# trifectatechfoundation/zlib-rs

Measured on NVIDIA H100. Metric: deflate_level6_raw_input_throughput_silesia_small_tar, higher is better.
Workload: dtype u8

## Files before the change

### __graft_entry__.py

```python
import os
import subprocess
import sys

ROOT = os.path.dirname(os.path.abspath(__file__))
if ROOT not in sys.path:
    sys.path.insert(0, ROOT)
sys.path.insert(0, os.path.join(ROOT, "tests"))


def build():
    subprocess.check_call(["make", "-C", os.path.join(ROOT, "zlib_rs_b200", "csrc"), "-j8"])
    subprocess.check_call(["make", "-C", os.path.join(ROOT, "oracle")])
    subprocess.check_call(["make", "-C", os.path.join(ROOT, "oracle"), "ref"])
    subprocess.check_call(["make", "-C", os.path.join(ROOT, "tests", "hostmodel")])
    subprocess.check_call(["make", "-C", os.path.join(ROOT, "tests", "shardmodel")])
    subprocess.check_call(["make", "-C", os.path.join(ROOT, "tests", "membermodel")])
    subprocess.check_call(["make", "-C", os.path.join(ROOT, "tests", "bgzfmodel")])
    subprocess.check_call(["make", "-C", os.path.join(ROOT, "tests", "c_client")])
    import zlib_rs_b200
    zlib_rs_b200.lib()


def smoke():
    import zlib
    import zlib_rs_b200 as Z
    import oracle_lib as O
    from corpus import synthetic_mix
    d = synthetic_mix(300000, seed=1)
    out = Z.compress2(d, 6)
    assert out == O.compress(d, 6)[1], "GPU deflate differs from the oracle"
    assert zlib.decompress(out) == d
    assert Z.uncompress(out, len(d)) == d
    assert Z.crc32(d) == O.crc32(d) and Z.adler32(d) == O.adler32(d)
    print("smoke ok: %d -> %d bytes, bit-exact vs oracle" % (len(d), len(out)))


if __name__ == "__main__":
    build()
    if len(sys.argv) > 1 and sys.argv[1] == "smoke":
        smoke()
```

### zlib_rs_b200/csrc/zb_core.h

```cpp
#pragma once
#include <stdint.h>

#if defined(__CUDACC__)
#define ZB_HD __host__ __device__ __forceinline__
#define ZB_HDN __host__ __device__
#else
#define ZB_HD inline
#define ZB_HDN
#endif

namespace zb {

constexpr uint32_t kWSize = 32768;
constexpr uint32_t kMaxDist = kWSize - 262;
constexpr uint32_t kMinLookahead = 262;
constexpr uint32_t kT0 = 2 * kWSize - 262;
constexpr uint32_t kMaxMatch = 258;
constexpr uint32_t kLitBufsize = 16384;
constexpr uint32_t kBlockSyms = kLitBufsize - 1;
constexpr uint32_t kTailZone = 1024;
constexpr uint32_t kMSafe = 640;
constexpr uint32_t kPad = 1024;

struct LevelParams {
    uint32_t good, lazy, nice, chain;
    uint32_t early_exit;
};
ZB_HD LevelParams level_params(int level)
{
    switch (level) {
    case 3: return {4, 6, 16, 6, 1};
    case 4: return {4, 12, 32, 24, 1};
    case 5: return {8, 16, 32, 32, 0};
    default: return {8, 16, 128, 128, 0};
    }
}

ZB_HD uint32_t hash_u32(uint32_t v) { return (v * 2654435761u) >> 16; }

struct FullWin {
    ZB_HD uint32_t wsize() const { return kWSize; }
    ZB_HD uint32_t maxdist() const { return kMaxDist; }
    ZB_HD uint32_t t0() const { return kT0; }
};
struct DynWin {
    uint32_t w;
    ZB_HD uint32_t wsize() const { return w; }
    ZB_HD uint32_t maxdist() const { return w - kMinLookahead; }
    ZB_HD uint32_t t0() const { return 2 * w - kMinLookahead; }
};
template <class WN>
ZB_HD uint32_t wbase_w(const WN &wn, uint32_t p) { return p <= wn.t0() ? 0u : wn.wsize() * (1u + (p - wn.t0() - 1u) / wn.wsize()); }

ZB_HD uint32_t wbase(uint32_t p) { return p <= kT0 ? 0u : kWSize * (1u + (p - kT0 - 1u) / kWSize); }

// ... 271 lines not shown
```

### zlib_rs_b200/csrc/zb_engine.cu

```cuda
#include <cuda_runtime.h>
#include <stdio.h>
#include <stdlib.h>
#include <string.h>
#include <new>
#include "../../include/zb_engine.h"
#include "zb_kernels.cuh"
#include "zb_engine_internal.h"

namespace zb {

constexpr uint32_t kSlowSub9 = 24576;
constexpr uint32_t kTailTiles = 2;
constexpr uint32_t kTailSub = 512;

thread_local char g_err[256] = "";

static void set_err(const char *what, cudaError_t e)
{
    snprintf(g_err, sizeof g_err, "%s: %s", what, cudaGetErrorString(e));
}

#define CK(call)                                                  \
    do {                                                          \
        cudaError_t e_ = (call);                                  \
        if (e_ != cudaSuccess) { set_err(#call, e_); return ZB_E_CUDA; } \
    } while (0)

__global__ void k_match(JobBufs);
__global__ void k_skip(JobBufs);
__global__ void k_nxt(JobBufs);
__global__ void k_path_tiles(JobBufs);
__global__ void k_path_chain(JobBufs, uint32_t, uint32_t);
__global__ void k_path_groups(JobBufs, uint32_t, uint32_t, uint4 *, uint32_t *);
__global__ void k_path_chain2(JobBufs, uint32_t, uint32_t, const uint4 *, uint32_t *, uint32_t *);
__global__ void k_path_mark(JobBufs, const uint32_t *, const uint32_t *);
__global__ void k_iter_lists(JobBufs, uint32_t *, uint32_t *, uint32_t);
__global__ void k_emit(JobBufs);
__global__ void k_holes(JobBufs, uint32_t);
__global__ void k_holes_cmp(JobBufs, uint32_t, uint32_t);
__global__ void k_tail(JobBufs);
__global__ void k_block_hist(JobBufs, uint32_t *);
__global__ void k_build_blocks(JobBufs, const uint32_t *);
__global__ void k_scan_blocks(JobBufs);
__global__ void k_encode(JobBufs);
__global__ void k_finish(JobBufs, const uint32_t *);
__global__ void k_literal_syms(JobBufs);
__global__ void k_stored(JobBufs);
__global__ void k_links2_std(JobBufs, uint32_t);
__global__ void k_links2_roll(JobBufs, uint32_t);
__global__ void k_links_fix_std(JobBufs);
__global__ void k_links_fix_roll(JobBufs);
__global__ void k_slow(JobBufs);
__global__ void k_rle(JobBufs);
__global__ void k_emit_slow(JobBufs);
__global__ void k_tail_slow(JobBufs);
__global__ void k_serial_low(JobBufs);
__global__ void k_links_dict_ghost(JobBufs, uint32_t *);
__global__ void k_links_dict_ghost_apply(JobBufs, const uint32_t *);
__global__ void k_bgzf_setup(BgzfJob, uint64_t);
__global__ void k_serial_low_members(JobBufs, BgzfJob);
__global__ void k_bgzf_medium(JobBufs, BgzfJob);
__global__ void k_bgzf_slow_steps(JobBufs, BgzfJob);
__global__ void k_bgzf_slow_walk(JobBufs, BgzfJob);
__global__ void k_bgzf_hist(JobBufs, BgzfJob, uint32_t *);
__global__ void k_bgzf_build(JobBufs, BgzfJob, const uint32_t *);
__global__ void k_bgzf_size(JobBufs, BgzfJob);
__global__ void k_bgzf_scan(JobBufs, BgzfJob);
__global__ void k_bgzf_encode(JobBufs, BgzfJob);
// ... 193 lines not shown
    RES(S_PCNT, ((size_t)N + 16) * 4, pcnt, uint32_t *)
    RES(S_SYMIDX, ((size_t)N + 16) * 4, symidx, uint32_t *)
    RES(S_PHEAD, (size_t)npt * kPathHead * 8, phead, uint2 *)
    RES(S_TENTRY, (size_t)npt * 4, tile_entry, uint32_t *)
    RES(S_TSYMB, (size_t)npt * 4, tile_symbase, uint32_t *)
    RES(S_MARKN, (size_t)npt + 16, mark_needed, uint8_t *)
    const uint32_t nlists = npt * (kPathTile / kPathSub);
    RES(S_LLIST, (size_t)nlists * kLongPerSub * 4, long_list, uint32_t *)
    RES(S_LCNT, (size_t)nlists * 4, long_cnt, uint32_t *)
    RES(S_TDIRTY, (size_t)nmt + 16, tile_dirty, uint8_t *)
    RES(S_SYMS, ((size_t)N + 64) * sizeof(Sym), syms, Sym *)
    RES(S_SYMB, 40000 * 4, sym_base, uint32_t *)
    RES(S_BMAP, (size_t)nmt * 8192, bucket_map, uint32_t *)
    RES(S_LR, npad * 2, Lr, uint16_t *)
    RES(S_KEYS, npad * 2, keys, uint16_t *)
    RES(S_LLAST, (size_t)nmt * 65536 * 2, link_last, uint16_t *)
    RES(S_CSTATE, (size_t)(npt + 1) * 16, chain_state, uint4 *)
    uint32_t chainG = 16;
    while ((uint64_t)chainG * chainG < npt) chainG += 8;
    const uint32_t chain_groups = (npt + chainG - 1) / chainG;
    const uint32_t chain2_smem = chainG * kPathHead * 8 + chain_groups * kPathHead * 16 + chainG * 8;
    const bool chain2 = chain2_smem <= kChain2MaxSmem;
    if ((rc = reserve(S_GFN, (size_t)chain_groups * kPathHead * 16 + ((size_t)npt + 4) * 4, &p)) != ZB_OK) return rc;
    uint4 *d_gfn = static_cast<uint4 *>(p);
    uint32_t *d_mark_cnt = reinterpret_cast<uint32_t *>(d_gfn + (size_t)chain_groups * kPathHead);
    uint32_t *d_mark_list = d_mark_cnt + 4;
    auto launch_chain = [&](uint32_t first_tile) {
        if (chain2) {
            k_path_groups<<<chain_groups, 1024, chainG * kPathHead * 8, st>>>(jb, npt, chainG, d_gfn, d_mark_cnt);
            k_path_chain2<<<chain_groups, 1024, chain2_smem, st>>>(jb, npt, chainG, d_gfn, d_mark_list, d_mark_cnt);
            launches++;
        } else k_path_chain<<<1, 1024, kChainSmemBytes, st>>>(jb, npt, first_tile);
    };
    auto launch_mark = [&](uint32_t grid) {
        if (chain2) k_path_mark<<<grid < npt ? grid : npt, 1024, kPathSmemBytes, st>>>(jb, d_mark_list, d_mark_cnt);
        else k_path_mark<<<npt, 1024, kPathSmemBytes, st>>>(jb, nullptr, nullptr);
    };
    uint32_t *d_lists;
    const uint32_t max_list = N / 512 + 2;
    if ((rc = reserve(S_LISTS, ((size_t)max_list + npt + nmt + 8) * 4, &p)) != ZB_OK) return rc;
    d_lists = static_cast<uint32_t *>(p);
    RES(S_HDIFF, (size_t)nwords * 8, hdiff, uint32_t *)
    jb.hdiff_words = nwords;
    RES(S_HCOARSE, (size_t)(N >> 10) + 16, hcoarse, uint8_t *)
    RES(S_MCHG, (((size_t)N >> 8) + 16) * 4 + 64, mchg, uint8_t *)
    RES(S_BLOCKS, (size_t)max_blocks * sizeof(BlockDesc), blocks, BlockDesc *)
    RES(S_BBASE, (size_t)max_blocks * 4, block_base, uint32_t *)
    uint32_t *d_freq;
    if ((rc = reserve(S_FREQ, (size_t)max_blocks * 320 * 4, &p)) != ZB_OK) return rc;
    d_freq = static_cast<uint32_t *>(p);
    uint8_t *d_out;
    if (dst_dev && dst_cap >= out_cap) d_out = static_cast<uint8_t *>(dst);
    else { if ((rc = reserve(S_OUT, out_cap + 16, &p)) != ZB_OK) return rc; d_out = static_cast<uint8_t *>(p); }
    jb.out = d_out;
    jb.out_cap = out_cap;
    void *d_ck;
    const size_t ck_bytes = ((size_t)N / 16384 + 16) * 8;
    if ((rc = reserve(S_CK, ck_bytes, &d_ck)) != ZB_OK) return rc;
#undef RES
    jb.info = d_info;
    jb.level = (uint32_t)level;
    jb.strategy_fixed = strategy == 4;
    const bool lf_zero = strategy >= 2;
    jb.wrap = wrap;
    jb.hdr_len = wrap == 1 ? 2 : wrap == 2 ? 10 : 0;
    jb.huffman_only = strategy == 2 && level != 0;
// ... 89 lines not shown
                cudaStreamWaitEvent(st, evc[k], 0);
                if (k + 1 < up_chunks) t_hi = up_len[k] >= 64 ? (uint32_t)((up_len[k] - 64) / kLinkTile) : 0;
            }
            if (t_hi <= t_done) continue;
            if (roll) k_links2_roll<<<t_hi - t_done, 1024, kLinks2SmemBytes, st>>>(jb, t_done);
            else k_links2_std<<<t_hi - t_done, 1024, kLinks2SmemBytes, st>>>(jb, t_done);
            if (k) launches++;
            t_done = t_hi;
        }
        if (chunked_upload) cudaStreamWaitEvent(st, evk, 0);
    };
    uint32_t iters = 0;
    if (level == 0) {
        const uint32_t nb = n_in == 0 ? 1 : (uint32_t)((n_in + 65534) / 65535);
        k_stored<<<nb, 256, 0, st>>>(jb);
        launches++;
        k_finish<<<1, 32, 0, st>>>(jb, d_check);
        launches++;
    } else {
        if (jb.huffman_only) {
            k_literal_syms<<<(uint32_t)(n_in / 256 + 1), 256, 0, st>>>(jb);
            launches++;
        } else if (jb.serial_mode) {
            iters = 1;
            pbegin();
            k_serial_low<<<1, 32, jb.serial_mode == 2 ? kSerialSmemBytes : kSerialSmemQuick, st>>>(jb);
            launches++;
            pend(1, 1);
        } else {
            CK(cudaMemsetAsync(jb.holes, 0, (size_t)nwords * 4, st));
            CK(cudaMemsetAsync(jb.holes_new, 0, (size_t)nwords * 4, st));
            CK(cudaMemsetAsync(jb.tile_dirty, 1, nmt, st));
            CK(cudaMemsetAsync(jb.tile_entry, 0xee, (size_t)npt * 4, st));
            CK(cudaMemsetAsync(jb.M + N, 0, (size_t)kPad * 4, st));
            CK(cudaMemsetAsync(jb.L + N, 0, (size_t)kPad * 2, st));
            pbegin();
            if (jb.slow_mode == 2) {
            } else if (jb.slow_mode && jb.sp.slow) {
                links_tiles(true);
                k_links_fix_roll<<<N / 256 + 1, 256, 0, st>>>(jb);
                launches += 2;
            } else {
                links_tiles(false);
                k_links_fix_std<<<N / 256 + 1, 256, 0, st>>>(jb);
                launches += 2;
                if (dstart >= 3 && n_in) {
                    uint32_t *d_first = reinterpret_cast<uint32_t *>(d_check) + 2;
                    CK(cudaMemsetAsync(d_first, 0xff, 4, st));
                    k_links_dict_ghost<<<(kMaxDist + 255) / 256, 256, 0, st>>>(jb, d_first);
                    k_links_dict_ghost_apply<<<1, 32, 0, st>>>(jb, d_first);
                    launches += 2;
                }
            }
            if (!jb.slow_mode) CK(cudaMemcpyAsync(jb.Lr, jb.L, npad * 2, cudaMemcpyDeviceToDevice, st));
            pend(0, 1);
            if (jb.slow_mode) {
                if (n_in > 0) {
                    iters = 1;
                    pbegin();
                    if (jb.slow_mode == 2) k_rle<<<(N + 255) / 256, 256, 0, st>>>(jb);
                    else {
                        jb.match_sub = level >= 9 ? kSlowSub9 : level == 8 ? 4096u : 8192u;
                        k_slow<<<(N + jb.match_sub - 1) / jb.match_sub, 1024, (kWSize + jb.match_sub + kSlowAhead) * 3, st>>>(jb);
                    }
                    pend(1, 1);
                    if (profile) phase_ms[11] = phase_ms[1];
                    pbegin();
                    k_path_tiles<<<npt, 1024, kPathSmemBytes, st>>>(jb);
                    launch_chain(0);
                    launch_mark(npt);
                    pend(3, 3);
                    pbegin();
                    k_emit_slow<<<(N + 255) / 256, 256, 0, st>>>(jb);
                    pend(4, 1);
                    launches += 5;
                }
                pbegin();
                k_tail_slow<<<1, 32, 0, st>>>(jb);
                launches++;
                pend(5, 1);
            } else {
            if (jb.tail_start > 0) {
                uint32_t n_dirty = nmt;
                for (;;) {
                    iters++;
                    uint32_t mthreads = 1024;
                    if (iters == 1) jb.match_sub = 4096;
                    else if (n_dirty <= kTailTiles) { jb.match_sub = kTailSub; mthreads = 256; }
                    else {
                        const uint64_t per_cta = (uint64_t)n_dirty * kMatchTile / (4 * (uint64_t)device_sm_count());
                        jb.match_sub = per_cta >= 8192 ? 8192 : per_cta >= 4096 ? 4096 : per_cta >= 2048 ? 2048 : 1024;
                    }
                    uint32_t nsub = (N + jb.match_sub - 1) / jb.match_sub;
                    uint32_t n_ptiles = npt, first_ptile = 0;
                    jb.skip_list = nullptr;
                    jb.nxt_list = nullptr;
                    if (iters > 1) {
                        jb.skip_list = d_lists;
                        jb.nxt_list = d_lists + nmt + 8;
                        n_ptiles = h_info->n_ptiles ? h_info->n_ptiles : 1;
                        first_ptile = h_info->first_ptile;
                        nsub = (n_dirty ? n_dirty : 1) * (kMatchTile / jb.match_sub);
                        if (n_dirty) {
                            pbegin();
                            k_skip<<<n_dirty, 1024, kSkipSmemBytes, st>>>(jb);
                            pend(1, 1);
                            launches++;
                        }
                    }
                    const uint32_t msmem = (kWSize + jb.match_sub + 512) + (kWSize + jb.match_sub) * 2 +
                                           (iters > 1 ? ((kWSize + jb.match_sub) / 32 + 1) * 4 * 4 + 8192 : 64);
                    jb.use_bucket_map = iters > 1;
                    pbegin();
                    k_match<<<nsub, mthreads, msmem, st>>>(jb);
                    pend(1, 1);
                    if (profile && iters == 1) phase_ms[11] = phase_ms[1];
                    pbegin();
                    k_nxt<<<n_ptiles * (kPathTile / 1024), 1024, 0, st>>>(jb);
                    pend(2, 1);
                    pbegin();
                    k_path_tiles<<<n_ptiles, 1024, kPathSmemBytes, st>>>(jb);
                    launch_chain(first_ptile);
                    launch_mark(iters == 1 ? npt : 2 * n_ptiles + 16);
                    pend(3, 3);
                    pbegin();
                    k_holes<<<(nlists * kLongPerSub + 255) / 256, 256, 0, st>>>(jb, nlists);
                    k_holes_cmp<<<(nwords + 255) / 256, 256, 0, st>>>(jb, nwords, nmt);
                    pend(4, 2);
                    launches += 7;
                    k_iter_lists<<<1, 1024, 0, st>>>(jb, d_lists, d_lists + nmt + 8, npt);
                    launches++;
                    CK(cudaMemcpyAsync(h_info, d_info, sizeof(JobInfo), cudaMemcpyDeviceToHost, st));
                    CK(cudaStreamSynchronize(st));
                    if (h_info->error) { snprintf(g_err, sizeof g_err, "engine error flags 0x%x (parse)", h_info->error); return ZB_E_INTERNAL; }
                    if (getenv("ZB_DEBUG")) {
                        static unsigned long long last[3];
                        if (iters == 1) memset(last, 0, sizeof last);
                        const double ctas = (double)(h_info->dbg[0] - last[0]) + 1e-9;
                        fprintf(stderr, "iter %u dirty %u: ctas %llu stage %.1f walk %.1f kcyc/cta, holes_changed %u, sub %u first_tile %u chain %u\n",
                                iters, n_dirty, h_info->dbg[0] - last[0], (h_info->dbg[1] - last[1]) / 1e3 / ctas,
                                (h_info->dbg[2] - last[2]) / 1e3 / ctas, h_info->holes_changed, jb.match_sub, first_ptile, chain2 ? 2u : 1u);
                        memcpy(last, h_info->dbg, sizeof last);
                    }
                    if (!h_info->holes_changed) break;
                    n_dirty = h_info->n_dirty;
                    if (iters > N / 257u + 4096u) { snprintf(g_err, sizeof g_err, "hole iteration did not converge"); return ZB_E_INTERNAL; }
                }
            }
            CK(cudaEventRecord(evf, st));
            CK(cudaStreamWaitEvent(st2, evf, 0));
            k_tail<<<1, 32, 0, st2>>>(jb);
            launches++;
            CK(cudaEventRecord(evt, st2));
            if (jb.tail_start > 0) {
                pbegin();
                k_emit<<<(jb.tail_start + 255) / 256, 256, 0, st>>>(jb);
                launches++;
                pend(4, 1);
            }
            pbegin();
            CK(cudaStreamWaitEvent(st, evt, 0));
            pend(5, 1);
            }
        }
        CK(cudaMemcpyAsync(h_info, d_info, sizeof(JobInfo), cudaMemcpyDeviceToHost, st));
        CK(cudaStreamSynchronize(st));
        if (h_info->error) { snprintf(g_err, sizeof g_err, "engine error flags 0x%x (tail)", h_info->error); return ZB_E_INTERNAL; }
        const uint32_t nblocks = h_info->n_blocks;
        if (nblocks == 0 || nblocks > max_blocks) { snprintf(g_err, sizeof g_err, "bad block count %u", nblocks); return ZB_E_INTERNAL; }
        pbegin();
        k_block_hist<<<nblocks, 256, 0, st>>>(jb, d_freq);
        k_build_blocks<<<nblocks, 32, 0, st>>>(jb, d_freq);
        k_scan_blocks<<<1, 256, 0, st>>>(jb);
        pend(6, 3);
        pbegin();
        k_encode<<<nblocks, 1024, 0, st>>>(jb);
        k_finish<<<1, 32, 0, st>>>(jb, d_check);
        pend(7, 2);
        launches += 5;
    }
    CK(cudaMemcpyAsync(h_info, d_info, sizeof(JobInfo), cudaMemcpyDeviceToHost, st));
    CK(cudaStreamSynchronize(st));
    CK(cudaGetLastError());
    if (h_info->error) {
        if (h_info->error & 8u) return ZB_E_BUF;
        snprintf(g_err, sizeof g_err, "engine error flags 0x%x (encode)", h_info->error);
// ... 363 lines not shown
```

### zlib_rs_b200/csrc/zb_engine_internal.h

```cpp
#pragma once
#include <cuda_runtime.h>
#include <stddef.h>
#include <stdint.h>
#include "../../include/zb_engine.h"
#include "zb_kernels.cuh"

namespace zb {

extern thread_local char g_err[256];
size_t deflate_bound(size_t n);

enum { S_IN, S_L, S_HOLES, S_HOLESN, S_M, S_NXT, S_PEXIT, S_PCNT, S_SYMIDX, S_TENTRY, S_TSYMB, S_TDIRTY, S_SYMS, S_SYMB,
       S_BLOCKS, S_SCRATCH, S_FREQ, S_OUT, S_CK, S_INF0, S_INF1, S_PHEAD, S_SK, S_MARKN, S_LLIST, S_LCNT, S_BMAP, S_HDIFF, S_HCOARSE, S_CSTATE, S_LISTS, S_LR, S_LLAST, S_BBASE, S_MCHG, S_GFN, S_KEYS, S_SHARD,
       S_MEMT, S_MEMC,
       S_BGZF,
       S_COUNT };

struct ShardState {
    int phase = 0;
    JobBufs jb;
    uint32_t off = 0, S = 0, E = 0, total = 0;
    uint32_t bs = 0, npt = 0, O = 0, n = 0, blo = 0, nloc = 0;
    bool is_last = false, tables = false;
    uint4 *gfn = nullptr;
    uint32_t chainG = 0, chain_groups = 0, chain2_smem = 0;
    uint32_t freq_lo[320], freq_hi[320];
    zb_shard_span span;
};

struct Engine {
    static constexpr int kSlots = 41;
    struct Buf { void *p = nullptr; size_t cap = 0; };
    int device = -1;
    cudaStream_t st = nullptr, st2 = nullptr;
    cudaEvent_t evf = nullptr, evt = nullptr;
    cudaEvent_t ev0 = nullptr, ev1 = nullptr;
    static constexpr int kUpChunks = 8;
    cudaEvent_t evk = nullptr;
    cudaEvent_t evc[kUpChunks] = {nullptr};
    Buf bufs[kSlots];
    void *h_stage = nullptr;
    size_t h_stage_cap = 0;
    JobInfo *h_info = nullptr, *d_info = nullptr;
    uint32_t *d_check = nullptr;
    void *d_inf_state = nullptr, *h_inf_state = nullptr;
    uint32_t launches = 0;
    uint8_t h_prime = 0;
    static constexpr int kPhases = 12;
    bool profile = false;
    float phase_ms[kPhases] = {0};
    uint32_t phase_launches[kPhases] = {0};
    cudaEvent_t pev0 = nullptr, pev1 = nullptr;
    void pbegin();
    void pend(int phase, uint32_t nlaunch);

    int init(int dev);
    int inflate_init();
    ~Engine();
    int reserve(int slot, size_t bytes, void **out);
    int stage(size_t bytes);
    int deflate(const void *src, size_t n, bool src_dev, void *dst, size_t dst_cap, bool dst_dev, int level, int strategy,
                int window_bits, uint32_t flags, zb_deflate_result *res, const void *dict = nullptr, size_t dict_len = 0);
    int deflate_bgzf(const void *src, size_t n, bool src_dev, void *dst, size_t dst_cap, bool dst_dev, int level, zb_deflate_result *res);
    int inflate(const void *src, size_t n, bool src_dev, void *dst, size_t dst_cap, bool dst_dev, int window_bits,
// ... 19 lines not shown
```

### zlib_rs_b200/csrc/zb_kernels.cu

```cuda
#include "zb_kernels.cuh"

namespace zb {

__constant__ HuffTables c_tab;

cudaError_t upload_tables()
{
    HuffTables t;
    init_tables(t);
    return cudaMemcpyToSymbol(c_tab, &t, sizeof t);
}

struct GAcc {
    const uint8_t *data;
    uint32_t N;
    const uint16_t *L;
    const uint32_t *holes;
    const uint32_t *M;
    uint32_t w = kWSize;
    __device__ __forceinline__ uint32_t byte(uint32_t y) const
    {
        while (y >= N) {
            if (y < 2 * w) return 0;
            y -= w;
// ... 618 lines not shown
    uint32_t m1 = ((pt + 1) * kPathTile + kMacroReach - 1) / kMatchTile;
    if (m1 >= jb.nmt) m1 = jb.nmt - 1;
    bool d = false;
    for (uint32_t m = m0; m <= m1; m++) d = d || jb.tile_dirty[m];
    return d;
}

__global__ void __launch_bounds__(1024) k_nxt(JobBufs jb)
{
    constexpr uint32_t per = kPathTile / 1024;
    const uint32_t tile = jb.nxt_list ? jb.nxt_list[blockIdx.x / per] : blockIdx.x / per;
    if (!path_tile_dirty(jb, tile)) return;
    const uint32_t p = tile * kPathTile + (blockIdx.x % per) * 1024 + threadIdx.x;
    if (p >= jb.tail_start) return;
    if (jb.use_bucket_map) {
        const uint32_t old = jb.nxt[p];
        const uint32_t b0 = p >> 6, b1 = min(p + (old & 0xffffu), jb.N) >> 6;
        bool chg = false;
        for (uint32_t b = b0; b <= b1; b++) chg = chg || jb.mchg[b];
        if (!chg) return;
    }
    GAcc a{jb.in, jb.N, jb.L, jb.holes, jb.M, jb.wsize};
    const uint32_t long_len = 16 * jb.lp.lazy;
    uint32_t ns = 0, nlong = 0, lpos = 0, llen = 0;
    auto see = [&](const Sym &s) {
        if (s.dist && (uint32_t)s.lc + 3u > long_len) { nlong++; lpos = s.pos; llen = s.lc + 3u; }
    };
    const uint32_t np = jb.wsize == kWSize ? macro_step(a, p, jb.lp, jb.tail_start, see, &ns)
                                           : macro_step(a, p, jb.lp, jb.tail_start, see, &ns, DynWin{jb.wsize});
    const uint32_t delta = np - p;
    if (delta > 0xffffu || ns > 0xffu || delta == 0) atomicOr(&jb.info->error, 1u);
    if (nlong && (nlong != 1 || lpos + llen != np || (jb.lp.early_exit ? lpos != p : (llen != 257u && llen != 258u))))
        atomicOr(&jb.info->error, 16u);
    jb.nxt[p] = (delta & 0xffffu) | ((ns & 0xffu) << 16) | (nlong ? kNxtLong : 0u) | (llen == 258u ? kNxtLong258 : 0u) |
                (np >= jb.tail_start ? kNxtTail : 0u);
}

constexpr uint32_t kStuck = 0x80000000u;
__device__ __forceinline__ void path_subtile(const uint32_t *nx, uint32_t *ex, uint32_t *cn, uint32_t s0, uint32_t s1, uint32_t lane)
{
    for (int32_t b = (int32_t)s1 - 32; b >= (int32_t)s0; b -= 32) {
        const uint32_t p = (uint32_t)b + lane;
        const uint32_t v = nx[p];
        uint32_t t, c;
        if (v & kNxtTail) { t = kStuck | p; c = 0; }
        else { t = p + (v & 0xffffu); c = (v >> 16) & 0xffu; }
#pragma unroll
        for (int r = 0; r < 5; r++) {
            const bool inb = !(t & kStuck) && t < (uint32_t)b + 32u;
            const uint32_t src = inb ? t - (uint32_t)b : lane;
            const uint32_t t2 = __shfl_sync(0xffffffffu, t, src);
            const uint32_t c2 = __shfl_sync(0xffffffffu, c, src);
            if (inb) { t = t2; c += c2; }
        }
        if (!(t & kStuck) && t < s1) { c += cn[t]; t = ex[t]; }
        ex[p] = t;
        cn[p] = c;
        __syncwarp();
    }
}

constexpr uint32_t kPathSmem = kPathTile * 4 * 3;

__device__ __forceinline__ void path_load(const JobBufs &jb, uint32_t tbeg, uint32_t *nx)
{
    const uint4 *src = reinterpret_cast<const uint4 *>(jb.nxt + tbeg);
    uint4 *dst = reinterpret_cast<uint4 *>(nx);
#pragma unroll 4
    for (uint32_t g = threadIdx.x; g < kPathTile / 4; g += blockDim.x) {
        const uint32_t p = tbeg + 4 * g;
        uint4 v;
        if (p + 3 < jb.tail_start) v = src[g];
        else {
            const uint32_t t = kNxtTail | 1u;
            v.x = p < jb.tail_start ? jb.nxt[p] : t;
            v.y = p + 1 < jb.tail_start ? jb.nxt[p + 1] : t;
            v.z = p + 2 < jb.tail_start ? jb.nxt[p + 2] : t;
            v.w = t;
        }
        dst[g] = v;
    }
}

__global__ void __launch_bounds__(1024) k_path_tiles(JobBufs jb)
{
    extern __shared__ __align__(16) uint8_t smem[];
    uint32_t *nx = reinterpret_cast<uint32_t *>(smem);
    uint32_t *ex = nx + kPathTile;
    uint32_t *cn = ex + kPathTile;
    const uint32_t tile = jb.nxt_list ? jb.nxt_list[blockIdx.x] : blockIdx.x;
    const uint32_t tbeg = tile * kPathTile;
    if (!path_tile_dirty(jb, tile)) return;
    path_load(jb, tbeg, nx);
    __syncthreads();
    const uint32_t warp = threadIdx.x >> 5, lane = threadIdx.x & 31;
    constexpr uint32_t kExitSub = 1024, nsub = kPathTile / kExitSub;
    for (uint32_t s = warp; s < nsub; s += blockDim.x / 32) path_subtile(nx, ex, cn, s * kExitSub, (s + 1) * kExitSub, lane);
    __syncthreads();
    for (int32_t j = (int32_t)nsub - 2; j >= 0; j--) {
        for (uint32_t i = threadIdx.x; i < kExitSub; i += blockDim.x) {
            const uint32_t p = (uint32_t)j * kExitSub + i;
            uint32_t t = ex[p];
            if (!(t & kStuck) && t < kPathTile) { cn[p] += cn[t]; ex[p] = ex[t]; }
        }
        __syncthreads();
    }
    for (uint32_t i = threadIdx.x; i < kPathTile; i += blockDim.x) {
        const uint32_t p = tbeg + i;
        const uint32_t t = ex[i];
        const uint32_t xa = (t & kStuck) ? (kStuck | (tbeg + (t & ~kStuck))) : tbeg + t;
        if (p < jb.tail_start) {
            jb.pexit[p] = xa;
            jb.pcnt[p] = cn[i];
        }
        if (i < kPathHead) jb.phead[(size_t)tile * kPathHead + i] = make_uint2(xa, cn[i]);
    }
}

constexpr uint32_t kChainChunk = kChainChunkTiles;
__global__ void __launch_bounds__(1024) k_path_chain(JobBufs jb, uint32_t ntiles, uint32_t first_tile)
{
    extern __shared__ __align__(16) uint8_t smem[];
    uint2 *hd = reinterpret_cast<uint2 *>(smem);
    __shared__ uint32_t s_e, s_base, s_done, s_tail;
    __shared__ uint32_t c_entry[kChainChunk], c_base[kChainChunk];
// ... 111 lines not shown
                if (f.z) { s.done = 1; s.tail = f.w; }
            }
            s_st = s; s_j = j;
        }
        __syncthreads();
        const uint32_t j = s_j;
        if (j >= g) break;
        chain_stage_heads(jb, hd, j * G, G);
        __syncthreads();
        if (threadIdx.x == 0) {
            ChainState s = s_st;
            chain_walk_group<false>(jb, hd, j * G, G, s, nullptr, nullptr);
            s_st = s; s_j = j + 1;
        }
        __syncthreads();
    }
    const uint32_t t0 = g * G, nt = min(G, ntiles - t0);
    chain_stage_heads(jb, hd, t0, nt);
    __syncthreads();
    if (threadIdx.x == 0) {
        ChainState s = s_st;
        chain_walk_group<true>(jb, hd, t0, nt, s, c_entry, c_base);
        if (g == gridDim.x - 1) {
            uint32_t tail_entry = s.tail;
            if (!s.done) { tail_entry = s.e; if (s.e < jb.tail_start) atomicOr(&jb.info->error, 2u); }
            jb.info->tail_entry = tail_entry;
            jb.info->n_mid_syms = s.base;
        }
    }
    __syncthreads();
    for (uint32_t k = threadIdx.x; k < nt; k += blockDim.x) {
        const uint32_t t = t0 + k;
        jb.tile_symbase[t] = c_base[k];
        const bool mn = (jb.tile_entry[t] != c_entry[k]) || path_tile_dirty(jb, t);
        jb.mark_needed[t] = mn;
        jb.tile_entry[t] = c_entry[k];
        if (mn) mark_list[atomicAdd(mark_cnt, 1u)] = t;
    }
}

__global__ void __launch_bounds__(1024) k_path_mark(JobBufs jb, const uint32_t *list, const uint32_t *list_cnt)
{
    extern __shared__ __align__(16) uint8_t smem[];
    uint32_t *nx = reinterpret_cast<uint32_t *>(smem);
    uint32_t *ex = nx + kPathTile;
    uint32_t *cn = ex + kPathTile;
    __shared__ uint32_t sub_entry[kPathTile / kPathSub], sub_base[kPathTile / kPathSub];
    constexpr uint32_t nsub = kPathTile / kPathSub;
    const uint32_t count = list ? *list_cnt : gridDim.x;
    for (uint32_t b = blockIdx.x; b < count; b += gridDim.x) {
        const uint32_t tile = list ? list[b] : b;
        const uint32_t tbeg = tile * kPathTile;
        if (!jb.mark_needed[tile]) continue;
        const uint32_t entry = jb.tile_entry[tile];
        if (threadIdx.x < nsub) jb.long_cnt[tile * nsub + threadIdx.x] = 0;
        if (entry == 0xffffffffu) {
            for (uint32_t i = threadIdx.x; i < kPathTile; i += blockDim.x)
                if (tbeg + i < jb.tail_start) jb.symidx[tbeg + i] = 0;
            continue;
        }
        __syncthreads();
        path_load(jb, tbeg, nx);
        __syncthreads();
        const uint32_t warp = threadIdx.x >> 5, lane = threadIdx.x & 31;
        for (uint32_t s = warp; s < nsub; s += blockDim.x / 32) path_subtile(nx, ex, cn, s * kPathSub, (s + 1) * kPathSub, lane);
        __syncthreads();
        if (threadIdx.x == 0) {
            uint32_t cur = entry - tbeg, cbase = 0;
            for (uint32_t j = 0; j < nsub; j++) {
                if (!(cur & kStuck) && cur < (j + 1) * kPathSub) {
                    sub_entry[j] = cur;
                    sub_base[j] = cbase;
                    cbase += cn[cur];
                    cur = ex[cur];
                } else sub_entry[j] = 0xffffffffu;
            }
        }
        __syncthreads();
        for (uint32_t i = threadIdx.x; i < kPathTile; i += blockDim.x) ex[i] = 0;
        __syncthreads();
        if (threadIdx.x < nsub) {
            const uint32_t s = threadIdx.x;
            uint32_t p = sub_entry[s];
            if (p != 0xffffffffu) {
                uint32_t idx = sub_base[s], nlong = 0;
                const uint32_t s1 = (s + 1) * kPathSub;
                uint32_t *ll = jb.long_list + (size_t)(tile * nsub + s) * kLongPerSub;
                while (p < s1) {
                    const uint32_t v = nx[p];
                    if (v & kNxtTail) break;
                    if (v & kNxtLong) {
                        if (nlong < kLongPerSub) ll[nlong++] = tbeg + p;
                        else atomicOr(&jb.info->error, 32u);
                    }
                    ex[p] = idx + 1;
                    idx += (v >> 16) & 0xffu;
                    p += v & 0xffffu;
                }
                jb.long_cnt[tile * nsub + s] = nlong;
            }
        }
        __syncthreads();
        for (uint32_t i = threadIdx.x; i < kPathTile; i += blockDim.x)
            if (tbeg + i < jb.tail_start) jb.symidx[tbeg + i] = ex[i];
    }
}

__global__ void __launch_bounds__(256) k_holes(JobBufs jb, uint32_t nlists)
{
    const uint32_t t = blockIdx.x * blockDim.x + threadIdx.x;
    {
        const uint32_t nthr = gridDim.x * blockDim.x;
        for (uint32_t i = t; i < jb.nmt; i += nthr) jb.tile_dirty[i] = 0;
        for (uint32_t i = t; i < jb.nmt * 512; i += nthr) reinterpret_cast<uint4 *>(jb.bucket_map)[i] = make_uint4(0, 0, 0, 0);
        for (uint32_t i = t; i < (jb.N >> 10) + 16; i += nthr) jb.hcoarse[i] = 0;
        for (uint32_t i = t; i < (jb.N >> 8) + 16; i += nthr) reinterpret_cast<uint32_t *>(jb.mchg)[i] = 0;
        if (t == 0) jb.info->holes_changed = 0;
    }
    const uint32_t list = t / kLongPerSub, slot = t % kLongPerSub;
    if (list >= nlists || slot >= jb.long_cnt[list]) return;
    const uint32_t p = jb.long_list[(size_t)list * kLongPerSub + slot];
    const uint32_t v = jb.nxt[p], delta = v & 0xffffu;
    const uint32_t len = jb.lp.early_exit ? delta : ((v & kNxtLong258) ? 258u : 257u);
    const uint32_t pos = p + delta - len;
    uint32_t y0 = pos + 1, y1 = pos + len - 1;
    uint32_t *hn = jb.holes_new;
    while (y0 < y1) {
        const uint32_t w = y0 >> 5, lo = y0 & 31;
        const uint32_t n = min(32u - lo, y1 - y0);
        const uint32_t mask = (n == 32 ? 0xffffffffu : ((1u << n) - 1u)) << lo;
        atomicOr(&hn[w], mask);
        y0 += n;
    }
}

__global__ void __launch_bounds__(256) k_emit(JobBufs jb)
{
    const uint32_t p = blockIdx.x * blockDim.x + threadIdx.x;
    if (p >= jb.tail_start) return;
    const uint32_t idx = jb.symidx[p];
    if (!idx) return;
    GAcc a{jb.in, jb.N, jb.L, jb.holes, jb.M, jb.wsize};
    uint32_t k = jb.tile_symbase[p / kPathTile] + idx - 1, ns = 0;
    Sym *syms = jb.syms;
    auto put = [&](const Sym &s) { syms[k++] = s; };
    if (jb.wsize == kWSize) macro_step(a, p, jb.lp, jb.tail_start, put, &ns);
    else macro_step(a, p, jb.lp, jb.tail_start, put, &ns, DynWin{jb.wsize});
}

__global__ void __launch_bounds__(256) k_holes_cmp(JobBufs jb, uint32_t nwords, uint32_t nmtiles)
{
    __shared__ uint32_t sb[2048];
    const uint32_t w = blockIdx.x * blockDim.x + threadIdx.x;
    uint32_t a = 0, b = 0;
    if (w < nwords) { a = jb.holes[w]; b = jb.holes_new[w]; }
    const bool changed = a != b;
    if (!__syncthreads_or(changed)) {
        if (w < nwords) { jb.hdiff[w] = 0; jb.hdiff[jb.hdiff_words + w] = 0; jb.holes_new[w] = 0; }
        return;
    }
    for (uint32_t i = threadIdx.x; i < 2048; i += blockDim.x) sb[i] = 0;
    __syncthreads();
    if (w < nwords) {
        jb.hdiff[w] = b & ~a;
        jb.hdiff[jb.hdiff_words + w] = a & ~b;
        if (changed) {
            jb.hcoarse[w >> 5] = 1;
            const uint32_t t = (w * 32) / kMatchTile;
            jb.info->holes_changed = 1u;
            jb.tile_dirty[t] = 1;
            if (t + 1 < nmtiles) jb.tile_dirty[t + 1] = 1;
            jb.holes[w] = b;
            uint32_t diff = a ^ b;
            while (diff) {
                const uint32_t y = w * 32 + (__ffs(diff) - 1);
                diff &= diff - 1;
                if (y + 4 <= jb.N) {
                    const uint8_t *q = jb.in + y;
                    const uint32_t h = hash_u32((uint32_t)q[0] | ((uint32_t)q[1] << 8) | ((uint32_t)q[2] << 16) | ((uint32_t)q[3] << 24));
                    atomicOr(&sb[h >> 5], 1u << (h & 31));
                }
            }
        }
        jb.holes_new[w] = 0;
    }
    __syncthreads();
    uint32_t *bm = jb.bucket_map + (size_t)((blockIdx.x * blockDim.x * 32) / kMatchTile) * 2048;
    for (uint32_t i = threadIdx.x; i < 2048; i += blockDim.x) if (sb[i]) atomicOr(&bm[i], sb[i]);
}

__global__ void __launch_bounds__(1024) k_iter_lists(JobBufs jb, uint32_t *skip_list, uint32_t *path_list, uint32_t npt)
{
    __shared__ uint32_t s_wsum[32], s_total, s_first;
    const uint32_t tid = threadIdx.x, lane = tid & 31, warp = tid >> 5;
    if (tid == 0) s_first = 0xffffffffu;
    uint32_t base = 0;
    for (int which = 0; which < 2; which++) {
        const uint32_t n = which ? npt : jb.nmt;
        uint32_t *out = which ? path_list : skip_list;
        base = 0;
        for (uint32_t c0 = 0; c0 < n; c0 += 1024) {
            const uint32_t i = c0 + tid;
            const bool d = i < n && (which ? path_tile_dirty(jb, i) : jb.tile_dirty[i] != 0);
            const uint32_t m = __ballot_sync(0xffffffffu, d);
            __syncthreads();
            if (lane == 0) s_wsum[warp] = __popc(m);
            __syncthreads();
            if (warp == 0) {
                const uint32_t v = s_wsum[lane];
                uint32_t incl = v;
#pragma unroll
                for (int k = 1; k < 32; k <<= 1) { const uint32_t t = __shfl_up_sync(0xffffffffu, incl, k); if (lane >= (uint32_t)k) incl += t; }
                s_wsum[lane] = incl - v;
                if (lane == 31) s_total = incl;
            }
            __syncthreads();
            if (d) {
                out[base + s_wsum[warp] + __popc(m & ((1u << lane) - 1u))] = i;
                if (which) atomicMin(&s_first, i);
            }
            base += s_total;
        }
        __syncthreads();
        if (tid == 0) {
            if (which) { jb.info->n_ptiles = base; jb.info->first_ptile = s_first == 0xffffffffu ? 0u : s_first; }
            else jb.info->n_dirty = base;
// ... 695 lines not shown
```

### zlib_rs_b200/csrc/zb_kernels.cuh

```cuda
#pragma once
#include <cuda_runtime.h>
#include "zb_core.h"
#include "zb_huff.h"
#include "zb_slow.h"
#include "zb_bgzf.h"

namespace zb {

constexpr uint32_t kLinkTile = 32768;
constexpr uint32_t kMatchTile = 32768;
constexpr uint32_t kMatchSub = 8192;
constexpr uint32_t kPathTile = 16384;
constexpr uint32_t kPathSub = 256;
constexpr uint32_t kLongPerSub = 4;
constexpr uint32_t kPathHead = 64;
constexpr uint32_t kChainChunkTiles = 320;
constexpr uint32_t kNxtTail = 0x80000000u;
constexpr uint32_t kNxtLong = 0x40000000u;
constexpr uint32_t kNxtLong258 = 0x20000000u;
constexpr uint32_t kSymsPerThread = 16;
constexpr uint32_t kSlowAhead = 1024;

__device__ __forceinline__ uint32_t sld_u8(uint32_t a) { uint32_t v; asm volatile("ld.shared.u8 %0, [%1];" : "=r"(v) : "r"(a)); return v; }
__device__ __forceinline__ uint32_t sld_u16(uint32_t a) { uint32_t v; asm volatile("ld.shared.u16 %0, [%1];" : "=r"(v) : "r"(a)); return v; }
__device__ __forceinline__ uint32_t sld_u32(uint32_t a) { uint32_t v; asm volatile("ld.shared.u32 %0, [%1];" : "=r"(v) : "r"(a)); return v; }
__device__ __forceinline__ uint32_t sld_u32u(uint32_t a)
{
    const uint32_t al = a & ~3u;
    return __funnelshift_r(sld_u32(al), sld_u32(al + 4), (a & 3u) * 8u);
}

struct JobInfo {
    uint32_t n_mid_syms;
    uint32_t tail_entry;
    uint32_t n_syms;
    uint32_t final_base;
    uint32_t holes_changed;
    uint32_t n_dirty, n_ptiles, first_ptile;
    uint32_t n_blocks;
    uint32_t data_type;
    uint32_t error;
    uint64_t total_bits;
    uint64_t out_bytes;
    uint32_t adler;
    uint64_t marker_byte;
    unsigned long long dbg[3];
};

struct JobBufs {
    const uint8_t *in;
    uint32_t N;
    uint32_t start;
    uint32_t tail_start;
    uint16_t *L;
    uint16_t *SK;
    uint32_t *hdiff;
    uint32_t hdiff_words;
    uint8_t *hcoarse;
    uint8_t *mchg;
    uint32_t *holes;
    uint32_t *holes_new;
    uint32_t *M;
    uint32_t *nxt;
    uint32_t *pexit;
    uint32_t *pcnt;
    uint2 *phead;
    uint32_t *symidx;
    uint32_t *tile_entry;
    uint32_t *tile_symbase;
    uint8_t *tile_dirty;
    Sym *syms;
    uint32_t *sym_base;
    BlockDesc *blocks;
    TreeScratch *scratch;
    uint8_t *out;
    uint64_t out_cap;
    JobInfo *info;
    LevelParams lp;
    uint32_t level;
    uint32_t strategy_fixed;
    uint32_t wrap;
    uint32_t hdr_len;
    uint32_t xfl;
    uint32_t huffman_only;
    uint32_t match_sub;
    uint32_t nmt;
    uint8_t *mark_needed;
    uint32_t *long_list;
    uint32_t *long_cnt;
    SlowParams sp;
    uint32_t slow_mode;
    uint16_t *link_last;
    uint16_t *Lr;
    uint16_t *keys;
    const uint32_t *skip_list;
    const uint32_t *nxt_list;
    uint4 *chain_state;
    uint32_t *bucket_map;
    uint32_t use_bucket_map;
    uint32_t not_last;
    uint32_t end_mode;
    uint32_t prime_bits;
    uint32_t block_syms;
    uint32_t serial_mode;
    uint32_t *block_base;
    uint32_t wsize;
    uint32_t cinfo;
};

struct BgzfCtl {
    uint32_t count;
    uint32_t error;
    uint32_t n_blocks;
    uint32_t n_syms;
    uint32_t data_type;
    uint32_t pad;
    uint64_t out_bytes;
};
struct BgzfJob {
    uint32_t nm;
    uint64_t *moff;
    uint32_t *mlen;
    uint32_t *mcrc;
    uint32_t *mbytes;
    uint64_t *mout;
    uint32_t *mstored;
    JobInfo *minfo;
    BgzfCtl *ctl;
};

cudaError_t upload_tables();
int device_sm_count();
cudaError_t launch_adler32(const uint8_t *d_buf, uint64_t len, uint32_t start, void *d_scratch, size_t scratch_bytes, uint32_t *d_out,
                           cudaStream_t st);
cudaError_t launch_crc32(const uint8_t *d_buf, uint64_t len, uint32_t start, void *d_scratch, size_t scratch_bytes, uint32_t *d_out,
                         cudaStream_t st);
cudaError_t launch_crc32_segments(const uint8_t *d_buf, const uint64_t *d_off, const uint32_t *d_len, uint32_t nseg, uint32_t *d_crc,
                                  cudaStream_t st);
cudaError_t launch_crc32_join(const uint32_t *d_crc, const uint32_t *d_len, const uint32_t *d_count, uint32_t *d_out, cudaStream_t st);

// ... 2 lines not shown
```

Measured before the change: 1.592.

## Incrementally rewalk parse path for small changes instead of full path recompute

In later hole-iteration rounds that touch few path tiles, k_nxt records the positions on the path whose next pointer changed. A single-block k_path_rewalk kernel then re-follows only those segments, patching symidx and the long lists and marking tiles stale. This replaces the per-iteration path_tiles/chain/mark launches, and a full path recompute runs once after convergence. A fallback to the full path handles overflow or long walks, at the cost of extra buffers, memsets and a second pass when the fallback triggers.

After: 1.637 (median of 6 runs). +2.8%, better.

```diff
diff --git a/__graft_entry__.py b/__graft_entry__.py
--- a/__graft_entry__.py
+++ b/__graft_entry__.py
@@ -13,6 +13,7 @@
     subprocess.check_call(["make", "-C", os.path.join(ROOT, "oracle")])
     subprocess.check_call(["make", "-C", os.path.join(ROOT, "oracle"), "ref"])
     subprocess.check_call(["make", "-C", os.path.join(ROOT, "tests", "hostmodel")])
+    subprocess.check_call(["make", "-C", os.path.join(ROOT, "tests", "rewalkmodel")])
     subprocess.check_call(["make", "-C", os.path.join(ROOT, "tests", "shardmodel")])
     subprocess.check_call(["make", "-C", os.path.join(ROOT, "tests", "membermodel")])
     subprocess.check_call(["make", "-C", os.path.join(ROOT, "tests", "bgzfmodel")])
diff --git a/zlib_rs_b200/csrc/zb_core.h b/zlib_rs_b200/csrc/zb_core.h
--- a/zlib_rs_b200/csrc/zb_core.h
+++ b/zlib_rs_b200/csrc/zb_core.h
@@ -21,6 +21,8 @@
 constexpr uint32_t kTailZone = 1024;
 constexpr uint32_t kMSafe = 640;
 constexpr uint32_t kPad = 1024;
+constexpr uint32_t kRewalkCap = 1024;
+constexpr uint32_t kRewalkSteps = 64;
 
 struct LevelParams {
     uint32_t good, lazy, nice, chain;
diff --git a/zlib_rs_b200/csrc/zb_engine.cu b/zlib_rs_b200/csrc/zb_engine.cu
--- a/zlib_rs_b200/csrc/zb_engine.cu
+++ b/zlib_rs_b200/csrc/zb_engine.cu
@@ -34,6 +34,7 @@
 __global__ void k_path_groups(JobBufs, uint32_t, uint32_t, uint4 *, uint32_t *);
 __global__ void k_path_chain2(JobBufs, uint32_t, uint32_t, const uint4 *, uint32_t *, uint32_t *);
 __global__ void k_path_mark(JobBufs, const uint32_t *, const uint32_t *);
+__global__ void k_path_rewalk(JobBufs);
 __global__ void k_iter_lists(JobBufs, uint32_t *, uint32_t *, uint32_t);
 __global__ void k_emit(JobBufs);
 __global__ void k_holes(JobBufs, uint32_t);
@@ -293,6 +294,14 @@
             launches++;
         } else k_path_chain<<<1, 1024, kChainSmemBytes, st>>>(jb, npt, first_tile);
     };
+    constexpr uint32_t kRewalkTiles = 128;
+    const bool path_inc = chain2 && !jb.slow_mode && jb.tail_start > 0;
+    if (path_inc) {
+        if ((rc = reserve(S_PATHINC, (size_t)nwords * 4 + (size_t)kRewalkCap * 4 + npt + 16, &p)) != ZB_OK) return rc;
+        jb.pchg = static_cast<uint32_t *>(p);
+        jb.rw_list = jb.pchg + nwords;
+        jb.path_stale = reinterpret_cast<uint8_t *>(jb.rw_list + kRewalkCap);
+    }
     auto launch_mark = [&](uint32_t grid) {
         if (chain2) k_path_mark<<<grid < npt ? grid : npt, 1024, kPathSmemBytes, st>>>(jb, d_mark_list, d_mark_cnt);
         else k_path_mark<<<npt, 1024, kPathSmemBytes, st>>>(jb, nullptr, nullptr);
@@ -448,6 +457,10 @@
             CK(cudaMemsetAsync(jb.holes_new, 0, (size_t)nwords * 4, st));
             CK(cudaMemsetAsync(jb.tile_dirty, 1, nmt, st));
             CK(cudaMemsetAsync(jb.tile_entry, 0xee, (size_t)npt * 4, st));
+            if (path_inc) {
+                CK(cudaMemsetAsync(jb.pchg, 0, (size_t)nwords * 4, st));
+                CK(cudaMemsetAsync(jb.path_stale, 0, npt, st));
+            }
             CK(cudaMemsetAsync(jb.M + N, 0, (size_t)kPad * 4, st));
             CK(cudaMemsetAsync(jb.L + N, 0, (size_t)kPad * 2, st));
             pbegin();
@@ -496,8 +509,30 @@
                 launches++;
                 pend(5, 1);
             } else {
+            bool final_marks = false;
             if (jb.tail_start > 0) {
                 uint32_t n_dirty = nmt;
+                bool stale = false;
+                bool rewalk_ok = path_inc;
+                auto full_path = [&](uint32_t n_ptiles, uint32_t first_ptile, uint32_t mark_grid) {
+                    JobBufs jt = jb;
+                    if (stale) { jt.nxt_list = nullptr; n_ptiles = npt; }
+                    k_path_tiles<<<n_ptiles, 1024, kPathSmemBytes, st>>>(jt);
+                    launch_chain(first_ptile);
+                    launch_mark(mark_grid);
+                    stale = false;
+                };
+                auto holes_and_lists = [&]() {
+                    pbegin();
+                    k_holes<<<(nlists * kLongPerSub + 255) / 256, 256, 0, st>>>(jb, nlists);
+                    k_holes_cmp<<<(nwords + 255) / 256, 256, 0, st>>>(jb, nwords, nmt);
+                    pend(4, 2);
+                    k_iter_lists<<<1, 1024, 0, st>>>(jb, d_lists, d_lists + nmt + 8, npt);
+                    launches += 3;
+                    CK(cudaMemcpyAsync(h_info, d_info, sizeof(JobInfo), cudaMemcpyDeviceToHost, st));
+                    CK(cudaStreamSynchronize(st));
+                    return (int)ZB_OK;
+                };
                 for (;;) {
                     iters++;
                     uint32_t mthreads = 1024;
@@ -531,23 +566,32 @@
                     k_match<<<nsub, mthreads, msmem, st>>>(jb);
                     pend(1, 1);
                     if (profile && iters == 1) phase_ms[11] = phase_ms[1];
+                    const bool rewalk = rewalk_ok && iters > 1 && n_ptiles <= kRewalkTiles;
+                    jb.rewalk = rewalk;
                     pbegin();
                     k_nxt<<<n_ptiles * (kPathTile / 1024), 1024, 0, st>>>(jb);
                     pend(2, 1);
                     pbegin();
-                    k_path_tiles<<<n_ptiles, 1024, kPathSmemBytes, st>>>(jb);
-                    launch_chain(first_ptile);
-                    launch_mark(iters == 1 ? npt : 2 * n_ptiles + 16);
-                    pend(3, 3);
-                    pbegin();
-                    k_holes<<<(nlists * kLongPerSub + 255) / 256, 256, 0, st>>>(jb, nlists);
-                    k_holes_cmp<<<(nwords + 255) / 256, 256, 0, st>>>(jb, nwords, nmt);
-                    pend(4, 2);
-                    launches += 7;
-                    k_iter_lists<<<1, 1024, 0, st>>>(jb, d_lists, d_lists + nmt + 8, npt);
-                    launches++;
-                    CK(cudaMemcpyAsync(h_info, d_info, sizeof(JobInfo), cudaMemcpyDeviceToHost, st));
-                    CK(cudaStreamSynchronize(st));
+                    if (rewalk) {
+                        k_path_rewalk<<<1, 1024, 0, st>>>(jb);
+                        stale = true;
+                        launches += 3;
+                    } else {
+                        full_path(n_ptiles, first_ptile, iters == 1 ? npt : 2 * n_ptiles + 16);
+                        launches += 5;
+                    }
+                    pend(3, rewalk ? 1 : 3);
+                    if ((rc = holes_and_lists()) != ZB_OK) return rc;
+                    if (h_info->path_fallback) {
+                        if (h_info->path_fallback == 2) rewalk_ok = false;
+                        CK(cudaMemsetAsync(jb.pchg, 0, (size_t)nwords * 4, st));
+                        CK(cudaMemsetAsync(&d_info->path_fallback, 0, sizeof(uint32_t), st));
+                        pbegin();
+                        full_path(n_ptiles, first_ptile, 2 * n_ptiles + 16);
+                        pend(3, 3);
+                        launches += 3;
+                        if ((rc = holes_and_lists()) != ZB_OK) return rc;
+                    }
                     if (h_info->error) { snprintf(g_err, sizeof g_err, "engine error flags 0x%x (parse)", h_info->error); return ZB_E_INTERNAL; }
                     if (getenv("ZB_DEBUG")) {
                         static unsigned long long last[3];
@@ -562,12 +606,28 @@
                     n_dirty = h_info->n_dirty;
                     if (iters > N / 257u + 4096u) { snprintf(g_err, sizeof g_err, "hole iteration did not converge"); return ZB_E_INTERNAL; }
                 }
+                if (stale) {
+                    JobBufs jt = jb;
+                    jt.nxt_list = nullptr;
+                    pbegin();
+                    k_path_tiles<<<npt, 1024, kPathSmemBytes, st>>>(jt);
+                    launch_chain(0);
+                    pend(3, 2);
+                    launches += 2;
+                    final_marks = true;
+                }
             }
             CK(cudaEventRecord(evf, st));
             CK(cudaStreamWaitEvent(st2, evf, 0));
             k_tail<<<1, 32, 0, st2>>>(jb);
             launches++;
             CK(cudaEventRecord(evt, st2));
+            if (final_marks) {
+                pbegin();
+                launch_mark((uint32_t)device_sm_count());
+                pend(3, 1);
+                launches++;
+            }
             if (jb.tail_start > 0) {
                 pbegin();
                 k_emit<<<(jb.tail_start + 255) / 256, 256, 0, st>>>(jb);
diff --git a/zlib_rs_b200/csrc/zb_engine_internal.h b/zlib_rs_b200/csrc/zb_engine_internal.h
--- a/zlib_rs_b200/csrc/zb_engine_internal.h
+++ b/zlib_rs_b200/csrc/zb_engine_internal.h
@@ -14,6 +14,7 @@
        S_BLOCKS, S_SCRATCH, S_FREQ, S_OUT, S_CK, S_INF0, S_INF1, S_PHEAD, S_SK, S_MARKN, S_LLIST, S_LCNT, S_BMAP, S_HDIFF, S_HCOARSE, S_CSTATE, S_LISTS, S_LR, S_LLAST, S_BBASE, S_MCHG, S_GFN, S_KEYS, S_SHARD,
        S_MEMT, S_MEMC,
        S_BGZF,
+       S_PATHINC,
        S_COUNT };
 
 struct ShardState {
@@ -29,7 +30,7 @@
 };
 
 struct Engine {
-    static constexpr int kSlots = 41;
+    static constexpr int kSlots = 42;
     struct Buf { void *p = nullptr; size_t cap = 0; };
     int device = -1;
     cudaStream_t st = nullptr, st2 = nullptr;
diff --git a/zlib_rs_b200/csrc/zb_kernels.cu b/zlib_rs_b200/csrc/zb_kernels.cu
--- a/zlib_rs_b200/csrc/zb_kernels.cu
+++ b/zlib_rs_b200/csrc/zb_kernels.cu
@@ -674,8 +674,17 @@
     if (delta > 0xffffu || ns > 0xffu || delta == 0) atomicOr(&jb.info->error, 1u);
     if (nlong && (nlong != 1 || lpos + llen != np || (jb.lp.early_exit ? lpos != p : (llen != 257u && llen != 258u))))
         atomicOr(&jb.info->error, 16u);
-    jb.nxt[p] = (delta & 0xffffu) | ((ns & 0xffu) << 16) | (nlong ? kNxtLong : 0u) | (llen == 258u ? kNxtLong258 : 0u) |
-                (np >= jb.tail_start ? kNxtTail : 0u);
+    const uint32_t nv = (delta & 0xffffu) | ((ns & 0xffu) << 16) | (nlong ? kNxtLong : 0u) | (llen == 258u ? kNxtLong258 : 0u) |
+                        (np >= jb.tail_start ? kNxtTail : 0u);
+    if (jb.use_bucket_map && nv != jb.nxt[p]) {
+        if (jb.path_stale) jb.path_stale[tile] = 1;
+        if (jb.rewalk && (jb.symidx[p] != 0 || p == jb.info->tail_entry)) {
+            atomicOr(&jb.pchg[p >> 5], 1u << (p & 31));
+            const uint32_t i = atomicAdd(&jb.info->rw_count, 1u);
+            if (i < kRewalkCap) jb.rw_list[i] = p;
+        }
+    }
+    jb.nxt[p] = nv;
 }
 
 constexpr uint32_t kStuck = 0x80000000u;
@@ -732,7 +741,7 @@
     uint32_t *cn = ex + kPathTile;
     const uint32_t tile = jb.nxt_list ? jb.nxt_list[blockIdx.x] : blockIdx.x;
     const uint32_t tbeg = tile * kPathTile;
-    if (!path_tile_dirty(jb, tile)) return;
+    if (!path_tile_dirty(jb, tile) && !(jb.path_stale && jb.path_stale[tile])) return;
     path_load(jb, tbeg, nx);
     __syncthreads();
     const uint32_t warp = threadIdx.x >> 5, lane = threadIdx.x & 31;
@@ -910,7 +919,7 @@
     for (uint32_t k = threadIdx.x; k < nt; k += blockDim.x) {
         const uint32_t t = t0 + k;
         jb.tile_symbase[t] = c_base[k];
-        const bool mn = (jb.tile_entry[t] != c_entry[k]) || path_tile_dirty(jb, t);
+        const bool mn = (jb.tile_entry[t] != c_entry[k]) || path_tile_dirty(jb, t) || (jb.path_stale && jb.path_stale[t]);
         jb.mark_needed[t] = mn;
         jb.tile_entry[t] = c_entry[k];
         if (mn) mark_list[atomicAdd(mark_cnt, 1u)] = t;
@@ -931,6 +940,7 @@
         const uint32_t tbeg = tile * kPathTile;
         if (!jb.mark_needed[tile]) continue;
         const uint32_t entry = jb.tile_entry[tile];
+        if (jb.path_stale && threadIdx.x == 0) jb.path_stale[tile] = 0;
         if (threadIdx.x < nsub) jb.long_cnt[tile * nsub + threadIdx.x] = 0;
         if (entry == 0xffffffffu) {
             for (uint32_t i = threadIdx.x; i < kPathTile; i += blockDim.x)
@@ -984,8 +994,115 @@
     }
 }
 
+__global__ void __launch_bounds__(1024) k_path_rewalk(JobBufs jb)
+{
+    __shared__ uint32_t s_c[kRewalkCap], s_r[kRewalkCap];
+    __shared__ uint16_t s_next[kRewalkCap], s_live[kRewalkCap];
+    __shared__ uint8_t s_on[kRewalkCap];
+    __shared__ uint32_t s_fail, s_nlive, s_tail;
+    const uint32_t tid = threadIdx.x, lane = tid & 31, warp = tid >> 5;
+    const uint32_t m = jb.info->rw_count, old_tail = jb.info->tail_entry;
+    if (m > kRewalkCap) {
+        if (tid == 0) { jb.info->rw_count = 0; jb.info->path_fallback = 1; }
+        return;
+    }
+    uint32_t P = 1;
+    while (P < m) P <<= 1;
+    if (tid == 0) { s_fail = 0; s_tail = old_tail; }
+    if (tid < P) s_c[tid] = tid < m ? jb.rw_list[tid] : 0xffffffffu;
+    if (tid < kRewalkCap) s_on[tid] = 0;
+    __syncthreads();
+    for (uint32_t k = 2; k <= P; k <<= 1)
+        for (uint32_t j = k >> 1; j > 0; j >>= 1) {
+            const uint32_t i = tid, l = i ^ j;
+            if (i < P && l > i) {
+                const uint32_t a = s_c[i], b = s_c[l];
+                if ((a > b) == ((i & k) == 0)) { s_c[i] = b; s_c[l] = a; }
+            }
+            __syncthreads();
+        }
+    uint32_t nodes[kRewalkSteps], nn = 0, c = 0, r = 0xffffffffu;
+    if (tid < m) {
+        c = s_c[tid];
+        uint32_t p = c, v = jb.nxt[c];
+#pragma unroll 1
+        for (uint32_t step = 0; step < kRewalkSteps; step++) {
+            if (v & kNxtTail) { r = kStuck | p; break; }
+            nodes[nn++] = p;
+            p += v & 0xffffu;
+            const uint32_t si = jb.symidx[p], cw = jb.pchg[p >> 5];
+            v = jb.nxt[p];
+            if ((si != 0 || p == old_tail) && !((cw >> (p & 31)) & 1u)) { r = p; break; }
+        }
+        if (r == 0xffffffffu) s_fail = 2;
+        s_r[tid] = r;
+    }
+    __syncthreads();
+    if (tid < m) {
+        atomicAnd(&jb.pchg[c >> 5], ~(1u << (c & 31)));
+        uint32_t lo = tid + 1, hi = m;
+        while (lo < hi) { const uint32_t mid = (lo + hi) >> 1; if (s_c[mid] < r) lo = mid + 1; else hi = mid; }
+        s_next[tid] = (uint16_t)lo;
+    }
+    if (tid == 0) {
+        jb.info->rw_count = 0;
+        if (s_fail) jb.info->path_fallback = s_fail;
+    }
+    __syncthreads();
+    if (s_fail) return;
+    if (tid == 0) {
+        uint32_t nl = 0;
+        for (uint32_t i = 0; i < m; i = s_next[i]) {
+            s_on[i] = 1;
+            s_live[nl++] = (uint16_t)i;
+            if (s_r[i] & kStuck) { s_tail = s_r[i] & ~kStuck; break; }
+        }
+        s_nlive = nl;
+    }
+    __syncthreads();
+    const uint32_t new_tail = s_tail;
+    if (tid < m && s_on[tid]) {
+        const uint32_t hi = (r & kStuck) ? max(new_tail, old_tail) + 1 : r;
+        uint32_t q = c + 1;
+        for (; q < hi && (q & 3); q++) jb.symidx[q] = 0;
+        for (; q + 4 <= hi; q += 4) *reinterpret_cast<uint4 *>(jb.symidx + q) = make_uint4(0, 0, 0, 0);
+        for (; q < hi; q++) jb.symidx[q] = 0;
+        for (uint32_t k = 0; k < nn; k++) jb.symidx[nodes[k]] = 1;
+        if (r & kStuck) jb.symidx[new_tail] = 0;
+        for (uint32_t t = c / kPathTile; t <= (hi - 1) / kPathTile; t++) jb.path_stale[t] = 1;
+        s_r[tid] = hi;
+    }
+    __syncthreads();
+    const uint32_t nl = s_nlive;
+    for (uint32_t k = warp; k < nl; k += 32) {
+        const uint32_t i = s_live[k], c0 = s_c[i], hi = s_r[i];
+        for (uint32_t s = c0 / kPathSub; s <= (hi - 1) / kPathSub; s++) {
+            uint32_t si[kPathSub / 32], v[kPathSub / 32];
+#pragma unroll
+            for (uint32_t j = 0; j < kPathSub / 32; j++) {
+                const uint32_t q = s * kPathSub + j * 32 + lane;
+                si[j] = q < jb.tail_start ? jb.symidx[q] : 0;
+                v[j] = q < jb.tail_start ? jb.nxt[q] : 0;
+            }
+            uint32_t cnt = 0;
+            uint32_t *ll = jb.long_list + (size_t)s * kLongPerSub;
+#pragma unroll
+            for (uint32_t j = 0; j < kPathSub / 32; j++) {
+                const bool lg = si[j] && (v[j] & (kNxtLong | kNxtTail)) == kNxtLong;
+                const uint32_t bm = __ballot_sync(0xffffffffu, lg);
+                const uint32_t slot = cnt + __popc(bm & ((1u << lane) - 1u));
+                if (lg) { if (slot < kLongPerSub) ll[slot] = s * kPathSub + j * 32 + lane; else atomicOr(&jb.info->error, 32u); }
+                cnt += __popc(bm);
+            }
+            if (lane == 0) jb.long_cnt[s] = min(cnt, kLongPerSub);
+        }
+    }
+    if (tid == 0) jb.info->tail_entry = new_tail;
+}
+
 __global__ void __launch_bounds__(256) k_holes(JobBufs jb, uint32_t nlists)
 {
+    if (jb.info->path_fallback) return;
     const uint32_t t = blockIdx.x * blockDim.x + threadIdx.x;
     {
         const uint32_t nthr = gridDim.x * blockDim.x;
@@ -1029,6 +1146,7 @@
 __global__ void __launch_bounds__(256) k_holes_cmp(JobBufs jb, uint32_t nwords, uint32_t nmtiles)
 {
     __shared__ uint32_t sb[2048];
+    if (jb.info->path_fallback) return;
     const uint32_t w = blockIdx.x * blockDim.x + threadIdx.x;
     uint32_t a = 0, b = 0;
     if (w < nwords) { a = jb.holes[w]; b = jb.holes_new[w]; }
@@ -1070,6 +1188,7 @@
 __global__ void __launch_bounds__(1024) k_iter_lists(JobBufs jb, uint32_t *skip_list, uint32_t *path_list, uint32_t npt)
 {
     __shared__ uint32_t s_wsum[32], s_total, s_first;
+    if (jb.info->path_fallback) return;
     const uint32_t tid = threadIdx.x, lane = tid & 31, warp = tid >> 5;
     if (tid == 0) s_first = 0xffffffffu;
     uint32_t base = 0;
diff --git a/zlib_rs_b200/csrc/zb_kernels.cuh b/zlib_rs_b200/csrc/zb_kernels.cuh
--- a/zlib_rs_b200/csrc/zb_kernels.cuh
+++ b/zlib_rs_b200/csrc/zb_kernels.cuh
@@ -45,6 +45,8 @@
     uint32_t adler;
     uint64_t marker_byte;
     unsigned long long dbg[3];
+    uint32_t rw_count;
+    uint32_t path_fallback;
 };
 
 struct JobBufs {
@@ -106,6 +108,10 @@
     uint32_t *block_base;
     uint32_t wsize;
     uint32_t cinfo;
+    uint8_t *path_stale;
+    uint32_t *pchg;
+    uint32_t *rw_list;
+    uint32_t rewalk;
 };
 
 struct BgzfCtl {
```
